# alipay/PainlessInferenceAcceleration

Hardware: NVIDIA H100
Metric: accepted tokens/sec @ Llama-2-7B 64-draft/8-branch; mean accepted len/step (higher is better)
Workload: dtype bf16

## Files before the change

painlessinferenceacceleration_b200/csrc/fused_ops.cu:

```cuda
#include <cuda_bf16.h>

#include "common.cuh"

namespace pia {
namespace fused {

__device__ __forceinline__ float bf(float x) { return __bfloat162float(__float2bfloat16_rn(x)); }

union Pack8 { uint4 u; __nv_bfloat16 h[8]; };

__device__ __forceinline__ Pack8 load_x8(const __nv_bfloat16 *x, const float *parts, int n_parts, long long part_stride,
                                         long long off) {
  Pack8 a;
  if (parts == nullptr) { a.u = *reinterpret_cast<const uint4 *>(x + off); return a; }
  float acc[8] = {0.f, 0.f, 0.f, 0.f, 0.f, 0.f, 0.f, 0.f};
  for (int s = 0; s < n_parts; ++s) {
    const float4 lo = *reinterpret_cast<const float4 *>(parts + s * part_stride + off);
    const float4 hi = *reinterpret_cast<const float4 *>(parts + s * part_stride + off + 4);
    acc[0] += lo.x; acc[1] += lo.y; acc[2] += lo.z; acc[3] += lo.w;
    acc[4] += hi.x; acc[5] += hi.y; acc[6] += hi.z; acc[7] += hi.w;
  }
#pragma unroll
  for (int j = 0; j < 8; ++j) a.h[j] = __float2bfloat16_rn(acc[j]);
  return a;
}

__global__ void __launch_bounds__(512) k_rmsnorm(const __nv_bfloat16 *x, const float *parts, int n_parts,
                                                 long long part_stride, const __nv_bfloat16 *res_in,
                                                 const __nv_bfloat16 *w, float eps, int hidden,
                                                 __nv_bfloat16 *res_out, __nv_bfloat16 *y) {
  __shared__ float red[16];
  pdl_launch_dependents();
  pdl_wait();
  const int row = blockIdx.x, tid = threadIdx.x;
  const int nvec = hidden >> 3;
  const long long row_off = (long long)row * hidden;
  const uint4 *rv = res_in ? reinterpret_cast<const uint4 *>(res_in + (long long)row * hidden) : nullptr;
  uint4 *rov = res_out ? reinterpret_cast<uint4 *>(res_out + (long long)row * hidden) : nullptr;
  float ss = 0.f;
  Pack8 keep[2];
  int cnt = 0;
  for (int v = tid; v < nvec; v += 512) {
    Pack8 a = load_x8(x, parts, n_parts, part_stride, row_off + v * 8);
    if (rv) {
      Pack8 r; r.u = rv[v];
#pragma unroll
      for (int j = 0; j < 8; ++j) a.h[j] = __float2bfloat16_rn(__bfloat162float(a.h[j]) + __bfloat162float(r.h[j]));
    }
    if (rov) rov[v] = a.u;
#pragma unroll
    for (int j = 0; j < 8; ++j) { const float f = __bfloat162float(a.h[j]); ss += f * f; }
    if (cnt < 2) keep[cnt] = a;
    ++cnt;
  }
#pragma unroll
  for (int o = 16; o > 0; o >>= 1) ss += __shfl_xor_sync(FULL, ss, o);
  if ((tid & 31) == 0) red[tid >> 5] = ss;
  __syncthreads();
  float tot = 0.f;
#pragma unroll
  for (int i = 0; i < 16; ++i) tot += red[i];
  const float inv = rsqrtf(tot / (float)hidden + eps);
  const uint4 *wv = reinterpret_cast<const uint4 *>(w);
  uint4 *yv = reinterpret_cast<uint4 *>(y + (long long)row * hidden);
  cnt = 0;
  for (int v = tid; v < nvec; v += 512) {
    Pack8 a;
    if (cnt < 2) a = keep[cnt];
    else {
      a = load_x8(x, parts, n_parts, part_stride, row_off + v * 8);
      if (rv) { Pack8 r; r.u = rv[v];
#pragma unroll
        for (int j = 0; j < 8; ++j) a.h[j] = __float2bfloat16_rn(__bfloat162float(a.h[j]) + __bfloat162float(r.h[j])); }
    }
    ++cnt;
    Pack8 ww; ww.u = wv[v];
    Pack8 o;
#pragma unroll
    for (int j = 0; j < 8; ++j) o.h[j] = __float2bfloat16_rn(__bfloat162float(ww.h[j]) * (__bfloat162float(a.h[j]) * inv));
    yv[v] = o.u;
  }
}

enum { ROPE_HALF = 0, ROPE_INTERLEAVED = 1, ROPE_HALF_F32 = 2 };
template <int kLayout>
__global__ void __launch_bounds__(256) k_rope_kv_append(const __nv_bfloat16 *qkv, const unsigned long long *mask,
                                                        int mask_words, pia_slots_t sl,
                                                        int hq, int hkv, int hd, const void *cos_t,
                                                        const void *sin_t, int max_pos, __nv_bfloat16 *q_out,
                                                        __nv_bfloat16 *kc, __nv_bfloat16 *vc, int max_seq,
                                                        int rotary_dim) {
  pdl_launch_dependents();
  pdl_wait();
  const int i = blockIdx.x;
  const int slot = i / sl.rows_per_slot, node = i % sl.rows_per_slot;
  const int n = sl.d_n[slot], P = sl.d_prefix_len[slot];
  const int pad_len = sl.d_pad_len ? sl.d_pad_len[slot] : 0;
  if (node >= n) return;
  kc += (long long)slot * sl.kv_slot_stride;
  vc += (long long)slot * sl.kv_slot_stride;
  int depth = -1;
  for (int w = 0; w < mask_words; ++w) depth += __popcll(mask[(long long)i * mask_words + w]);
  int pos = (P > pad_len ? P - pad_len : 0) + depth;
  if (pos < 0) pos = 0;
  if (pos >= max_pos) pos = max_pos - 1;
  const int half = hd >> 1, cpr = hd >> 3;
  const int row_elems = (hq + 2 * hkv) * hd;
  const __nv_bfloat16 *src = qkv + (long long)i * row_elems;
  const int cache_row = P + node;
  const int total = (hq + 2 * hkv) * cpr;
  for (int c = threadIdx.x; c < total; c += blockDim.x) {
    const int head = c / cpr, ch = c % cpr;
    const int d0 = ch * 8;
    Pack8 a; a.u = *reinterpret_cast<const uint4 *>(src + head * hd + d0);
    if (head < hq + hkv) {
      Pack8 o;
      const __nv_bfloat16 *cos_b = static_cast<const __nv_bfloat16 *>(cos_t);
      const __nv_bfloat16 *sin_b = static_cast<const __nv_bfloat16 *>(sin_t);
      if constexpr (kLayout == ROPE_INTERLEAVED) {
        o = a;
        if (d0 < rotary_dim) {
          const int rhalf = rotary_dim >> 1;
          union { uint2 u; __nv_bfloat16 h[4]; } cs, sn;
          cs.u = *reinterpret_cast<const uint2 *>(cos_b + (long long)pos * rhalf + (d0 >> 1));
          sn.u = *reinterpret_cast<const uint2 *>(sin_b + (long long)pos * rhalf + (d0 >> 1));
#pragma unroll
          for (int j = 0; j < 4; ++j) {
            const float x0 = __bfloat162float(a.h[2 * j]), x1 = __bfloat162float(a.h[2 * j + 1]);
            const float c = __bfloat162float(cs.h[j]), s = __bfloat162float(sn.h[j]);
            o.h[2 * j] = __float2bfloat16_rn(bf(x0 * c) + bf(-x1 * s));
            o.h[2 * j + 1] = __float2bfloat16_rn(bf(x1 * c) + bf(x0 * s));
          }
        }
      } else if constexpr (kLayout == ROPE_HALF_F32) {
        const int dp = d0 < half ? d0 + half : d0 - half;
        Pack8 b; b.u = *reinterpret_cast<const uint4 *>(src + head * hd + dp);
        const float *cf = static_cast<const float *>(cos_t) + (long long)pos * half + d0 % half;
        const float *sf = static_cast<const float *>(sin_t) + (long long)pos * half + d0 % half;
        float c[8], s[8];
        *reinterpret_cast<float4 *>(c) = *reinterpret_cast<const float4 *>(cf);
        *reinterpret_cast<float4 *>(c + 4) = *reinterpret_cast<const float4 *>(cf + 4);
        *reinterpret_cast<float4 *>(s) = *reinterpret_cast<const float4 *>(sf);
        *reinterpret_cast<float4 *>(s + 4) = *reinterpret_cast<const float4 *>(sf + 4);
#pragma unroll
        for (int j = 0; j < 8; ++j) {
          const float x = __bfloat162float(a.h[j]);
          const float r = d0 < half ? -__bfloat162float(b.h[j]) : __bfloat162float(b.h[j]);
          o.h[j] = __float2bfloat16_rn(__fadd_rn(__fmul_rn(x, c[j]), __fmul_rn(r, s[j])));
        }
      } else {
        const int dp = d0 < half ? d0 + half : d0 - half;
        Pack8 b; b.u = *reinterpret_cast<const uint4 *>(src + head * hd + dp);
        Pack8 cs, sn;
        const int f0 = d0 % half;
        cs.u = *reinterpret_cast<const uint4 *>(cos_b + (long long)pos * half + f0);
        sn.u = *reinterpret_cast<const uint4 *>(sin_b + (long long)pos * half + f0);
#pragma unroll
        for (int j = 0; j < 8; ++j) {
          const float x = __bfloat162float(a.h[j]);
          const float r = d0 < half ? -__bfloat162float(b.h[j]) : __bfloat162float(b.h[j]);
          o.h[j] = __float2bfloat16_rn(bf(x * __bfloat162float(cs.h[j])) + bf(r * __bfloat162float(sn.h[j])));
        }
      }
      if (head < hq) *reinterpret_cast<uint4 *>(q_out + ((long long)i * hq + head) * hd + d0) = o.u;
      else *reinterpret_cast<uint4 *>(kc + ((long long)(head - hq) * max_seq + cache_row) * hd + d0) = o.u;
    } else {
      *reinterpret_cast<uint4 *>(vc + ((long long)(head - hq - hkv) * max_seq + cache_row) * hd + d0) = a.u;
    }
  }
}

__global__ void __launch_bounds__(256) k_silu_mul(const __nv_bfloat16 *gu, int inter, __nv_bfloat16 *out) {
  pdl_launch_dependents();
  pdl_wait();
  const int row = blockIdx.y;
  const int v = blockIdx.x * 256 + threadIdx.x;
  if (v * 8 >= inter) return;
  Pack8 g, u, o;
  g.u = *reinterpret_cast<const uint4 *>(gu + (long long)row * 2 * inter + v * 8);
  u.u = *reinterpret_cast<const uint4 *>(gu + (long long)row * 2 * inter + inter + v * 8);
#pragma unroll
  for (int j = 0; j < 8; ++j) {
    const float x = __bfloat162float(g.h[j]);
    const float s = bf(x / (1.f + expf(-x)));
    o.h[j] = __float2bfloat16_rn(s * __bfloat162float(u.h[j]));
  }
  *reinterpret_cast<uint4 *>(out + (long long)row * inter + v * 8) = o.u;
}

__global__ void __launch_bounds__(256) k_embed_gather(const __nv_bfloat16 *table, const int *ids, const int *d_n,
                                                      int hidden, __nv_bfloat16 *out) {
  pdl_launch_dependents();
  pdl_wait();
  const int row = blockIdx.x;
  const int n = *d_n;
  const int nvec = hidden >> 3;
  uint4 *dst = reinterpret_cast<uint4 *>(out + (long long)row * hidden);
  if (row >= n) { for (int v = threadIdx.x; v < nvec; v += 256) dst[v] = make_uint4(0, 0, 0, 0); return; }
  const uint4 *src = reinterpret_cast<const uint4 *>(table + (long long)ids[row] * hidden);
  for (int v = threadIdx.x; v < nvec; v += 256) dst[v] = src[v];
}

}
}

using namespace pia;
using namespace pia::fused;

extern "C" int pia_rmsnorm(const void *d_x, const void *d_residual_in, const void *d_weight, float eps, int rows,
                           int hidden, void *d_residual_out, void *d_y, void *stream) {
  PIA_REQUIRE(d_x && d_weight && d_y && rows > 0 && hidden > 0 && hidden % 8 == 0, "bad rmsnorm arguments");
  PIA_CUDA_CHECK(launch_kernel(k_rmsnorm, dim3(rows), dim3(512), 0, (cudaStream_t)stream, (const __nv_bfloat16 *)d_x,
                              (const float *)nullptr, 0, 0ll, (const __nv_bfloat16 *)d_residual_in,
                              (const __nv_bfloat16 *)d_weight, eps, hidden, (__nv_bfloat16 *)d_residual_out,
                              (__nv_bfloat16 *)d_y));
  count_launch();
  return PIA_OK;
}

extern "C" int pia_rmsnorm_partials(const float *d_x_parts, int n_parts, int64_t part_stride, const void *d_residual_in,
                                    const void *d_weight, float eps, int rows, int hidden, void *d_residual_out,
                                    void *d_y, void *stream) {
  PIA_REQUIRE(d_x_parts && n_parts >= 1 && d_weight && d_y && rows > 0 && hidden > 0 && hidden % 8 == 0, "bad rmsnorm arguments");
  PIA_CUDA_CHECK(launch_kernel(k_rmsnorm, dim3(rows), dim3(512), 0, (cudaStream_t)stream,
                              (const __nv_bfloat16 *)nullptr, d_x_parts, n_parts, (long long)part_stride,
                              (const __nv_bfloat16 *)d_residual_in, (const __nv_bfloat16 *)d_weight, eps, hidden,
                              (__nv_bfloat16 *)d_residual_out, (__nv_bfloat16 *)d_y));
  count_launch();
  return PIA_OK;
}

template <int kLayout>
static int rope_kv_append(const void *d_qkv, const uint64_t *d_mask, int mask_words, const pia_slots_t *slots,
                          int n_q_heads, int n_kv_heads, int head_dim, const void *d_cos, const void *d_sin, int max_pos,
                          void *d_q_out, void *d_k_cache_layer, void *d_v_cache_layer, int max_seq, int rotary_dim,
                          void *stream) {
  PIA_REQUIRE(d_qkv && d_mask && slots && slots->d_n && slots->d_prefix_len && d_cos && d_sin && d_q_out &&
                  d_k_cache_layer && d_v_cache_layer, "null argument");
  PIA_REQUIRE(slots->batch >= 1 && slots->rows_per_slot >= 1 && slots->kv_slot_stride >= 0, "bad slot table");
  PIA_REQUIRE(head_dim % 16 == 0 && mask_words >= 1 && mask_words <= 2, "bad rope arguments");
  PIA_CUDA_CHECK(launch_kernel(k_rope_kv_append<kLayout>, dim3(slots->batch * slots->rows_per_slot), dim3(256), 0,
                              (cudaStream_t)stream, (const __nv_bfloat16 *)d_qkv, (const unsigned long long *)d_mask,
                              mask_words, *slots, n_q_heads, n_kv_heads, head_dim, d_cos, d_sin, max_pos,
                              (__nv_bfloat16 *)d_q_out,
                              (__nv_bfloat16 *)d_k_cache_layer, (__nv_bfloat16 *)d_v_cache_layer, max_seq, rotary_dim));
  count_launch();
  return PIA_OK;
}

extern "C" int pia_rope_kv_append(const void *d_qkv, const uint64_t *d_mask, int mask_words, const pia_slots_t *slots,
                                  int n_q_heads, int n_kv_heads, int head_dim, const void *d_cos, const void *d_sin,
                                  int max_pos, void *d_q_out, void *d_k_cache_layer, void *d_v_cache_layer, int max_seq,
                                  void *stream) {
  return rope_kv_append<ROPE_HALF>(d_qkv, d_mask, mask_words, slots, n_q_heads, n_kv_heads, head_dim, d_cos, d_sin,
                                   max_pos, d_q_out, d_k_cache_layer, d_v_cache_layer, max_seq, head_dim, stream);
}

extern "C" int pia_rope_f32_kv_append(const void *d_qkv, const uint64_t *d_mask, int mask_words, const pia_slots_t *slots,
                                      int n_q_heads, int n_kv_heads, int head_dim, const void *d_cos, const void *d_sin,
                                      int max_pos, void *d_q_out, void *d_k_cache_layer, void *d_v_cache_layer,
                                      int max_seq, void *stream) {
  return rope_kv_append<ROPE_HALF_F32>(d_qkv, d_mask, mask_words, slots, n_q_heads, n_kv_heads, head_dim, d_cos, d_sin,
                                       max_pos, d_q_out, d_k_cache_layer, d_v_cache_layer, max_seq, head_dim, stream);
}

extern "C" int pia_rope_interleaved_kv_append(const void *d_qkv, const uint64_t *d_mask, int mask_words,
                                              const pia_slots_t *slots, int n_q_heads, int n_kv_heads, int head_dim,
                                              const void *d_cos, const void *d_sin, int max_pos, void *d_q_out,
                                              void *d_k_cache_layer, void *d_v_cache_layer, int max_seq,
                                              int rotary_dim, void *stream) {
  PIA_REQUIRE(rotary_dim >= 8 && rotary_dim % 8 == 0 && rotary_dim <= head_dim,
              "bad rotary_dim: a positive multiple of 8, at most head_dim");
  return rope_kv_append<ROPE_INTERLEAVED>(d_qkv, d_mask, mask_words, slots, n_q_heads, n_kv_heads, head_dim, d_cos, d_sin, max_pos,
                              d_q_out, d_k_cache_layer, d_v_cache_layer, max_seq, rotary_dim, stream);
}

extern "C" int pia_silu_mul(const void *d_gate_up, int rows, int inter, void *d_out, void *stream) {
  PIA_REQUIRE(d_gate_up && d_out && rows > 0 && inter > 0 && inter % 8 == 0, "bad silu_mul arguments");
  dim3 grid((inter / 8 + 255) / 256, rows);
  PIA_CUDA_CHECK(launch_kernel(k_silu_mul, grid, dim3(256), 0, (cudaStream_t)stream, (const __nv_bfloat16 *)d_gate_up,
                              inter, (__nv_bfloat16 *)d_out));
  count_launch();
  return PIA_OK;
}

__global__ void __launch_bounds__(256) k_moe_combine(const __nv_bfloat16 *ye, const __nv_bfloat16 *w, int n_exp, int rows_cap,
                                                     int hidden, __nv_bfloat16 *out) {
  pdl_launch_dependents();
  pdl_wait();
  const int t = blockIdx.x;
  for (int v = threadIdx.x; v * 8 < hidden; v += blockDim.x) {
    Pack8 acc;
#pragma unroll
    for (int j = 0; j < 8; ++j) acc.h[j] = __float2bfloat16_rn(0.f);
    for (int e = 0; e < n_exp; ++e) {
      const float we = __bfloat162float(w[(long long)t * n_exp + e]);
      Pack8 y;
      y.u = *reinterpret_cast<const uint4 *>(ye + ((long long)e * rows_cap + t) * hidden + v * 8);
#pragma unroll
      for (int j = 0; j < 8; ++j)
        acc.h[j] = __float2bfloat16_rn(__bfloat162float(acc.h[j]) + bf(__bfloat162float(y.h[j]) * we));
    }
    *reinterpret_cast<uint4 *>(out + (long long)t * hidden + v * 8) = acc.u;
  }
}

extern "C" int pia_moe_combine(const void *d_expert_out, const void *d_weights, int n_experts, int rows, int rows_cap,
                               int hidden, void *d_out, void *stream) {
  PIA_REQUIRE(d_expert_out && d_weights && d_out && n_experts > 0 && rows > 0 && rows <= rows_cap && hidden % 8 == 0,
              "bad combine arguments");
  PIA_CUDA_CHECK(launch_kernel(k_moe_combine, dim3(rows), dim3(256), 0, (cudaStream_t)stream,
                              (const __nv_bfloat16 *)d_expert_out, (const __nv_bfloat16 *)d_weights, n_experts, rows_cap,
                              hidden, (__nv_bfloat16 *)d_out));
  count_launch();
  return PIA_OK;
}

__global__ void __launch_bounds__(256) k_moe_router(const __nv_bfloat16 *y, const __nv_bfloat16 *gate_w, int hidden,
                                                    int n_exp, int top_k, __nv_bfloat16 *dense) {
  __shared__ float s_logit[64];
  pdl_launch_dependents();
  pdl_wait();
  const int t = blockIdx.x, warp = threadIdx.x >> 5, lane = threadIdx.x & 31;
  const __nv_bfloat16 *yr = y + (long long)t * hidden;
  for (int e = warp; e < n_exp; e += 8) {
    const __nv_bfloat16 *wr = gate_w + (long long)e * hidden;
    float acc = 0.f;
    for (int v = lane; v * 8 < hidden; v += 32) {
      Pack8 a, w;
      a.u = *reinterpret_cast<const uint4 *>(yr + v * 8);
      w.u = *reinterpret_cast<const uint4 *>(wr + v * 8);
#pragma unroll
      for (int j = 0; j < 8; ++j) acc += __bfloat162float(a.h[j]) * __bfloat162float(w.h[j]);
    }
#pragma unroll
    for (int o = 16; o > 0; o >>= 1) acc += __shfl_xor_sync(FULL, acc, o);
    if (lane == 0) s_logit[e] = bf(acc);
  }
  __syncthreads();
  if (threadIdx.x == 0) {
    float mx = -INFINITY;
    for (int e = 0; e < n_exp; ++e) mx = fmaxf(mx, s_logit[e]);
    float den = 0.f, p[64];
    for (int e = 0; e < n_exp; ++e) { p[e] = expf(s_logit[e] - mx); den += p[e]; }
    for (int e = 0; e < n_exp; ++e) p[e] /= den;
    unsigned long long chosen = 0ull;
    float sum = 0.f;
    for (int k = 0; k < top_k; ++k) {
      int best = -1;
      for (int e = 0; e < n_exp; ++e)
        if (!((chosen >> e) & 1ull) && (best < 0 || p[e] > p[best])) best = e;
      chosen |= 1ull << best;
      sum += p[best];
    }
    for (int e = 0; e < n_exp; ++e)
      dense[(long long)t * n_exp + e] = __float2bfloat16_rn(((chosen >> e) & 1ull) ? p[e] / sum : 0.f);
  }
}

extern "C" int pia_moe_router(const void *d_y, const void *d_gate_weight, int rows, int hidden, int n_experts, int top_k,
                              void *d_dense_out, void *stream) {
  PIA_REQUIRE(d_y && d_gate_weight && d_dense_out && rows > 0 && hidden % 8 == 0 && n_experts >= 1 && n_experts <= 64 &&
                  top_k >= 1 && top_k <= n_experts, "bad router arguments");
  PIA_CUDA_CHECK(launch_kernel(k_moe_router, dim3(rows), dim3(256), 0, (cudaStream_t)stream, (const __nv_bfloat16 *)d_y,
                              (const __nv_bfloat16 *)d_gate_weight, hidden, n_experts, top_k, (__nv_bfloat16 *)d_dense_out));
  count_launch();
  return PIA_OK;
}

__global__ void __launch_bounds__(32) k_l2_prefetch(const char *base, long long n_ranges, long long stride,
                                                     long long range_bytes, int chunk, float bytes_per_ns) {
  const long long cpr = (range_bytes + chunk - 1) / chunk;
  const long long total = cpr * n_ranges;
  unsigned long long t0;
  asm volatile("mov.u64 %0, %%globaltimer;" : "=l"(t0));
  for (long long c = (long long)threadIdx.x * gridDim.x + blockIdx.x; c < total; c += (long long)blockDim.x * gridDim.x) {
    const long long k = c / n_ranges, r = c % n_ranges;
    const long long off = k * chunk;
    const long long left = range_bytes - off;
    const unsigned sz = (unsigned)(left < chunk ? left : chunk);
    if (bytes_per_ns > 0.f) {
      const unsigned long long due = t0 + (unsigned long long)((float)(c * chunk) / bytes_per_ns);
      unsigned long long now;
      asm volatile("mov.u64 %0, %%globaltimer;" : "=l"(now));
      while (now < due) {
        __nanosleep(64);
        asm volatile("mov.u64 %0, %%globaltimer;" : "=l"(now));
      }
    }
    asm volatile("cp.async.bulk.prefetch.L2.global [%0], %1;" ::"l"(base + r * stride + off), "r"(sz) : "memory");
  }
}

extern "C" int pia_l2_prefetch(const void *d_base, int64_t n_ranges, int64_t stride_bytes, int64_t range_bytes,
// ... 27 lines not shown
```

painlessinferenceacceleration_b200/csrc/gemm_ws.cu:

```cuda
#include <cuda.h>
#include <cuda_bf16.h>
#include <cuda_fp16.h>

#include <new>

#include "common.cuh"

namespace pia {
namespace gemm {

constexpr int BMW = 128;
constexpr int BK = 64;
constexpr int TOK = 64;
constexpr int NTHREADS = 288;
constexpr int PRODUCER_WARP = 8;
constexpr int W_BYTES = BMW * BK * 2, X_BYTES = TOK * BK * 2, STAGE_BYTES = W_BYTES + X_BYTES;
constexpr int XCH_BYTES = TOK * 64 * 2;
constexpr int smem_total(int nstage) { return nstage * STAGE_BYTES + 256 + XCH_BYTES + 1024; }
constexpr int ACC_OFF = 32 * 1024, ACC_LD = TOK + 4;
static_assert(ACC_OFF + BMW * ACC_LD * 4 <= 4 * STAGE_BYTES, "accumulator staging must fit in the pipeline stages");

__device__ __forceinline__ uint32_t smem_u32(const void *p) { return (uint32_t)__cvta_generic_to_shared(p); }
__device__ __forceinline__ void mbar_init(uint32_t bar, int count) {
  asm volatile("mbarrier.init.shared::cta.b64 [%0], %1;" ::"r"(bar), "r"(count));
}
__device__ __forceinline__ void mbar_arrive(uint32_t bar) {
  asm volatile("mbarrier.arrive.shared::cta.b64 _, [%0];" ::"r"(bar) : "memory");
}
__device__ __forceinline__ void mbar_expect_tx(uint32_t bar, uint32_t bytes) {
  asm volatile("mbarrier.arrive.expect_tx.shared::cta.b64 _, [%0], %1;" ::"r"(bar), "r"(bytes) : "memory");
}
__device__ __forceinline__ void mbar_wait(uint32_t bar, uint32_t parity) {
  uint32_t done;
  do {
    asm volatile(
        "{\n\t.reg .pred p;\n\t"
        "mbarrier.try_wait.parity.shared::cta.b64 p, [%1], %2;\n\t"
        "selp.u32 %0, 1, 0, p;\n\t}"
        : "=r"(done)
        : "r"(bar), "r"(parity)
        : "memory");
  } while (!done);
}
__device__ __forceinline__ void cluster_sync_all() {
  asm volatile("barrier.cluster.arrive.release.aligned;\n\tbarrier.cluster.wait.acquire.aligned;" ::: "memory");
}
__device__ __forceinline__ uint32_t map_to_cta(uint32_t local_smem_addr, uint32_t cta_rank) {
  uint32_t r;
  asm volatile("mapa.shared::cluster.u32 %0, %1, %2;" : "=r"(r) : "r"(local_smem_addr), "r"(cta_rank));
  return r;
}
__device__ __forceinline__ void st_cluster_f4(uint32_t addr, float a, float b, float c, float d) {
  asm volatile("st.shared::cluster.v4.f32 [%0], {%1, %2, %3, %4};" ::"r"(addr), "f"(a), "f"(b), "f"(c), "f"(d) : "memory");
}
__device__ __forceinline__ void tma_load_2d(uint32_t dst, const CUtensorMap *map, uint32_t bar, int c0, int c1) {
  asm volatile(
      "cp.async.bulk.tensor.2d.shared::cluster.global.mbarrier::complete_tx::bytes [%0], [%1, {%3, %4}], [%2];"
      ::"r"(dst), "l"(map), "r"(bar), "r"(c0), "r"(c1)
      : "memory");
}
__device__ __forceinline__ void tma_load_3d(uint32_t dst, const CUtensorMap *map, uint32_t bar, int c0, int c1, int c2) {
  asm volatile(
      "cp.async.bulk.tensor.3d.shared::cluster.global.mbarrier::complete_tx::bytes [%0], [%1, {%3, %4, %5}], [%2];"
      ::"r"(dst), "l"(map), "r"(bar), "r"(c0), "r"(c1), "r"(c2)
      : "memory");
}
__device__ __forceinline__ uint64_t kmajor_desc(uint32_t saddr) {
  uint64_t d = 0;
  d |= (uint64_t)((saddr >> 4) & 0x3FFF);
  d |= (uint64_t)1 << 16;
  d |= (uint64_t)(1024 >> 4) << 32;
  d |= (uint64_t)1 << 62;
  return d;
}
__device__ __forceinline__ void wgmma_fence() { asm volatile("wgmma.fence.sync.aligned;" ::: "memory"); }
__device__ __forceinline__ void wgmma_commit() { asm volatile("wgmma.commit_group.sync.aligned;" ::: "memory"); }
__device__ __forceinline__ void wgmma_wait_all() { asm volatile("wgmma.wait_group.sync.aligned 0;" ::: "memory"); }
__device__ __forceinline__ void fence_acc(float (&d)[32]) {
#pragma unroll
  for (int i = 0; i < 32; ++i) asm volatile("" : "+f"(d[i])::"memory");
}
__device__ __forceinline__ void wgmma_m64n64k16(float (&d)[32], uint64_t desc_a, uint64_t desc_b) {
  asm volatile(
      "{\n\t"
      "wgmma.mma_async.sync.aligned.m64n64k16.f32.bf16.bf16 "
      "{%0, %1, %2, %3, %4, %5, %6, %7, %8, %9, %10, %11, %12, %13, %14, %15, "
      "%16, %17, %18, %19, %20, %21, %22, %23, %24, %25, %26, %27, %28, %29, %30, %31}, %32, %33, 1, 1, 1, 0, 0;\n\t}"
      : "+f"(d[0]), "+f"(d[1]), "+f"(d[2]), "+f"(d[3]), "+f"(d[4]), "+f"(d[5]), "+f"(d[6]), "+f"(d[7]), "+f"(d[8]),
        "+f"(d[9]), "+f"(d[10]), "+f"(d[11]), "+f"(d[12]), "+f"(d[13]), "+f"(d[14]), "+f"(d[15]), "+f"(d[16]),
        "+f"(d[17]), "+f"(d[18]), "+f"(d[19]), "+f"(d[20]), "+f"(d[21]), "+f"(d[22]), "+f"(d[23]), "+f"(d[24]),
        "+f"(d[25]), "+f"(d[26]), "+f"(d[27]), "+f"(d[28]), "+f"(d[29]), "+f"(d[30]), "+f"(d[31])
      : "l"(desc_a), "l"(desc_b)
      : "memory");
}
__device__ __forceinline__ void mma_stage(float (&acc)[32], uint32_t wa, uint32_t xa) {
  wgmma_fence();
#pragma unroll
  for (int j = 0; j < BK / 16; ++j) wgmma_m64n64k16(acc, kmajor_desc(wa + j * 32), kmajor_desc(xa + j * 32));
  wgmma_commit();
  wgmma_wait_all();
  fence_acc(acc);
}
__device__ __forceinline__ int frag_row(int warp, int lane, int h) { return 16 * (warp & 3) + (lane >> 2) + 8 * h; }
__device__ __forceinline__ int frag_tok(int lane, int i) { return 8 * i + 2 * (lane & 3); }

struct Params {
  int N, K, n_split, chunks_per_split, n_chunks, rows, tiled;
  int groups, w_group_rows, x_group_chunks;
  long long out_group_stride;
  int cluster;
  int silu;
  int no_pdl;
  __nv_bfloat16 *out_bf16;
  float *out_f32;
};

template <int NSTAGE>
__global__ void __launch_bounds__(NTHREADS, NSTAGE <= 4 ? 2 : 1)
k_gemm_ws(const __grid_constant__ CUtensorMap map_w, const __grid_constant__ CUtensorMap map_x, Params p) {
  constexpr int SMEM_BAR = NSTAGE * STAGE_BYTES;
  extern __shared__ uint8_t smem_raw[];
  const uint32_t base = (smem_u32(smem_raw) + 1023u) & ~1023u;
  uint8_t *sm = smem_raw + (base - smem_u32(smem_raw));
  const int tid = threadIdx.x, warp = tid >> 5, lane = tid & 31;
  const uint32_t bar_full = base + SMEM_BAR, bar_empty = bar_full + 8 * NSTAGE;
  const int tile = p.cluster ? blockIdx.y : blockIdx.x, split = p.cluster ? blockIdx.x : blockIdx.y;
  const int n0 = tile * BMW;
  const int grp = blockIdx.z;
  const int xk0 = grp * p.x_group_chunks;
  const int c0 = split * p.chunks_per_split;
  int c1 = c0 + p.chunks_per_split;
  if (c1 > p.n_chunks) c1 = p.n_chunks;
  const int nch = c1 - c0;

  if (tid == 0) {
    for (int s = 0; s < NSTAGE; ++s) { mbar_init(bar_full + 8 * s, 1); mbar_init(bar_empty + 8 * s, 8); }
    asm volatile("fence.mbarrier_init.release.cluster;" ::: "memory");
  }
  __syncwarp();
  if (!p.no_pdl) pdl_launch_dependents();
  __syncthreads();

  if (warp == PRODUCER_WARP) {
    if (lane == 0) {
      auto load_w = [&](int i, int s) {
        const uint32_t wd = base + s * STAGE_BYTES;
        if (p.tiled) tma_load_3d(wd, &map_w, bar_full + 8 * s, 0, 0, tile * p.n_chunks + c0 + i);
        else tma_load_2d(wd, &map_w, bar_full + 8 * s, (c0 + i) * BK, grp * p.w_group_rows + n0);
      };
      const int pre = nch < NSTAGE ? nch : NSTAGE;
      for (int i = 0; i < pre; ++i) {
        mbar_expect_tx(bar_full + 8 * i, STAGE_BYTES);
        load_w(i, i);
      }
      pdl_wait();
      for (int i = 0; i < pre; ++i) tma_load_2d(base + i * STAGE_BYTES + W_BYTES, &map_x, bar_full + 8 * i, (xk0 + c0 + i) * BK, 0);
      for (int i = pre; i < nch; ++i) {
        const int s = i % NSTAGE, ph = (i / NSTAGE) & 1;
        mbar_wait(bar_empty + 8 * s, ph ^ 1);
        mbar_expect_tx(bar_full + 8 * s, STAGE_BYTES);
        load_w(i, s);
        tma_load_2d(base + s * STAGE_BYTES + W_BYTES, &map_x, bar_full + 8 * s, (xk0 + c0 + i) * BK, 0);
      }
    }
    __syncwarp();
    if (p.cluster) { cluster_sync_all(); cluster_sync_all(); }
    return;
  }

  pdl_wait();
  const int wg = warp >> 2;
  float acc[32];
#pragma unroll
  for (int j = 0; j < 32; ++j) acc[j] = 0.f;
  for (int i = 0; i < nch; ++i) {
    const int s = i % NSTAGE, ph = (i / NSTAGE) & 1;
    mbar_wait(bar_full + 8 * s, ph);
    const uint32_t wa = base + s * STAGE_BYTES, xa = wa + W_BYTES;
    mma_stage(acc, wa + wg * 64 * 128, xa);
    __syncwarp();
    if (lane == 0) mbar_arrive(bar_empty + 8 * s);
  }
  float *accs = reinterpret_cast<float *>(sm + ACC_OFF);
  asm volatile("bar.sync 2, 256;" ::: "memory");
#pragma unroll
  for (int h = 0; h < 2; ++h) {
    const int r = wg * 64 + frag_row(warp, lane, h);
#pragma unroll
    for (int i = 0; i < 8; ++i)
      *reinterpret_cast<float2 *>(accs + r * ACC_LD + frag_tok(lane, i)) = make_float2(acc[4 * i + 2 * h], acc[4 * i + 2 * h + 1]);
  }
  asm volatile("bar.sync 2, 256;" ::: "memory");
  if (wg == 1) {
    if (p.cluster) { cluster_sync_all(); cluster_sync_all(); }
    return;
  }

  const int q = warp;
  const int n = n0 + q * 32 + lane;
  uint32_t v[64];
  {
    const float4 *src = reinterpret_cast<const float4 *>(accs + (q * 32 + lane) * ACC_LD);
#pragma unroll
    for (int t = 0; t < 16; ++t) {
      const float4 a = src[t];
      v[4 * t] = __float_as_uint(a.x); v[4 * t + 1] = __float_as_uint(a.y);
      v[4 * t + 2] = __float_as_uint(a.z); v[4 * t + 3] = __float_as_uint(a.w);
    }
  }
  if (p.cluster) {
    const int cs = p.cluster, RS = BMW / cs;
    cluster_sync_all();
    {
      const int row = q * 32 + lane;
      const int owner = row / RS, rl = row % RS;
      const uint32_t dst = map_to_cta(base + (uint32_t)((split * 16) * RS + rl) * 16, owner);
#pragma unroll
      for (int tq = 0; tq < 16; ++tq)
        st_cluster_f4(dst + (uint32_t)(tq * RS) * 16, __uint_as_float(v[4 * tq]), __uint_as_float(v[4 * tq + 1]),
                      __uint_as_float(v[4 * tq + 2]), __uint_as_float(v[4 * tq + 3]));
    }
    cluster_sync_all();
    {
      const int e = warp * 32 + lane;
      const int rl = e % RS, tg = e / RS;
      const int qpt = RS / 8;
      const int n_out = n0 + split * RS + rl;
      const float4 *buf = reinterpret_cast<const float4 *>(sm);
      __nv_bfloat16 *ob = p.out_bf16 + grp * p.out_group_stride;
      if (n_out < p.N) {
        for (int tq = tg * qpt; tq < (tg + 1) * qpt; ++tq) {
          float4 a = buf[(0 * 16 + tq) * RS + rl];
          for (int src = 1; src < cs; ++src) {
            const float4 b = buf[(src * 16 + tq) * RS + rl];
            a.x += b.x; a.y += b.y; a.z += b.z; a.w += b.w;
          }
          const int t0 = 4 * tq;
          if (t0 < p.rows) ob[(long long)t0 * p.N + n_out] = __float2bfloat16_rn(a.x);
          if (t0 + 1 < p.rows) ob[(long long)(t0 + 1) * p.N + n_out] = __float2bfloat16_rn(a.y);
          if (t0 + 2 < p.rows) ob[(long long)(t0 + 2) * p.N + n_out] = __float2bfloat16_rn(a.z);
          if (t0 + 3 < p.rows) ob[(long long)(t0 + 3) * p.N + n_out] = __float2bfloat16_rn(a.w);
        }
      }
    }
  } else
  if (p.silu) {
    __nv_bfloat16 *xu = reinterpret_cast<__nv_bfloat16 *>(sm + SMEM_BAR + 256);
    __nv_bfloat16 *xg = xu + 32 * 64;
    const int rr = (q & 1) * 32 + lane;
    if (q >= 2) {
#pragma unroll
      for (int t = 0; t < 32; ++t) xu[t * 64 + rr] = __float2bfloat16_rn(__uint_as_float(v[t]));
    } else {
#pragma unroll
      for (int t = 0; t < 32; ++t) xg[t * 64 + rr] = __float2bfloat16_rn(__uint_as_float(v[32 + t]));
    }
    asm volatile("bar.sync 1, 128;" ::: "memory");
    const int col = tile * 64 + rr;
    const int inter = p.N >> 1;
    if (col < inter) {
      const int tb = q < 2 ? 0 : 32;
#pragma unroll
      for (int t = 0; t < 32; ++t) {
        if (tb + t < p.rows) {
          const float g = q < 2 ? __bfloat162float(__float2bfloat16_rn(__uint_as_float(v[t]))) : __bfloat162float(xg[t * 64 + rr]);
          const float u = q < 2 ? __bfloat162float(xu[t * 64 + rr]) : __bfloat162float(__float2bfloat16_rn(__uint_as_float(v[32 + t])));
          const float sg = __bfloat162float(__float2bfloat16_rn(g / (1.f + expf(-g))));
          p.out_bf16[(long long)(tb + t) * inter + col] = __float2bfloat16_rn(sg * u);
        }
      }
    }
  } else
  if (n < p.N) {
    if (p.n_split == 1) {
#pragma unroll
      for (int t = 0; t < TOK; ++t)
        if (t < p.rows) p.out_bf16[grp * p.out_group_stride + (long long)t * p.N + n] = __float2bfloat16_rn(__uint_as_float(v[t]));
    } else {
      float *o = p.out_f32 + (long long)split * TOK * p.N;
#pragma unroll
      for (int t = 0; t < TOK; ++t)
        if (t < p.rows) o[(long long)t * p.N + n] = __uint_as_float(v[t]);
    }
  }
}


struct SkParams {
  int N, n_tiles, n_chunks, rows, max_contrib;
  long long units;
  __nv_bfloat16 *out;
  float *ws;
  int *flags;
};

__device__ __forceinline__ long long sk_begin(long long b, long long U, int G) { return b * U / G; }
__device__ __forceinline__ int sk_cta_of(long long x, long long U, int G) {
  int b = (int)(x * G / U);
  while (b + 1 < G && sk_begin(b + 1, U, G) <= x) ++b;
  while (b > 0 && sk_begin(b, U, G) > x) --b;
  return b;
}

constexpr int SK_STAGES = 8;
constexpr int SK_SMEM_BAR = SK_STAGES * STAGE_BYTES;
constexpr int SK_SMEM_TOTAL = SK_SMEM_BAR + 256 + 1024;

__global__ void __launch_bounds__(NTHREADS, 1)
k_gemm_sk(const __grid_constant__ CUtensorMap map_w, const __grid_constant__ CUtensorMap map_x, SkParams p) {
  extern __shared__ uint8_t smem_raw[];
  const uint32_t base = (smem_u32(smem_raw) + 1023u) & ~1023u;
  const int tid = threadIdx.x, warp = tid >> 5, lane = tid & 31;
  const uint32_t bar_full = base + SK_SMEM_BAR, bar_empty = bar_full + 8 * SK_STAGES;
  const int G = gridDim.x, b = blockIdx.x;
  const long long u0 = sk_begin(b, p.units, G), u1 = sk_begin(b + 1, p.units, G);

  if (tid == 0) {
    for (int s = 0; s < SK_STAGES; ++s) { mbar_init(bar_full + 8 * s, 1); mbar_init(bar_empty + 8 * s, 8); }
    asm volatile("fence.mbarrier_init.release.cluster;" ::: "memory");
  }
  __syncwarp();
  pdl_launch_dependents();
  __syncthreads();
  pdl_wait();

  if (warp == PRODUCER_WARP) {
    if (lane == 0) {
      int i = 0;
      for (long long u = u0; u < u1; ++u, ++i) {
        const int tile = (int)(u / p.n_chunks), ch = (int)(u % p.n_chunks);
        const int s = i % SK_STAGES, ph = (i / SK_STAGES) & 1;
        mbar_wait(bar_empty + 8 * s, ph ^ 1);
        mbar_expect_tx(bar_full + 8 * s, STAGE_BYTES);
        const uint32_t wd = base + s * STAGE_BYTES, xd = wd + W_BYTES;
        tma_load_3d(wd, &map_w, bar_full + 8 * s, 0, 0, tile * p.n_chunks + ch);
// ... 614 lines not shown
```

painlessinferenceacceleration_b200/models/llama/modeling_llama.py:

```python
import glob
import json
import math
import os

import torch
from torch import nn

from ...common import ops
from ...common.pretrained_model import LookaheadPreTrainedModel


class LlamaRMSNorm(nn.Module):
    def __init__(self, hidden_size, eps=1e-6, device=None, dtype=None):
        super().__init__()
        self.weight = nn.Parameter(torch.ones(hidden_size, device=device, dtype=dtype))
        self.variance_epsilon = eps


class LlamaAttention(nn.Module):
    def __init__(self, cfg, device, dtype, qkv_bias=False):
        super().__init__()
        hd = cfg.hidden_size // cfg.num_attention_heads
        kv = getattr(cfg, 'num_key_value_heads', None) or cfg.num_attention_heads
        kw = dict(bias=False, device=device, dtype=dtype)
# ... 272 lines not shown
    def quantize_fp8(self):
        if self._fp8:
            return self
        self.fuse()
        for li, layer in enumerate(self.model.layers):
            for name, shape in self._fp8_weight_shapes(layer):
                if shape[-1] % 128 or shape[-2] % 128:
                    raise ValueError(f'layer {li} {name} {tuple(shape)}: fp8 weights need both dimensions divisible by 128')
        self._rt = None
        self.__dict__.pop('_tiled_weights', None)
        for layer in self.model.layers:
            self._quantize_layer(layer)
        self._fp8 = True
        return self

    def _quantize_layer(self, layer):
        a = layer.self_attn
        nq, nk = a.q_proj.weight.shape[0], a.k_proj.weight.shape[0]
        qkv = Fp8Linear(a.qkv_weight)
        a.qkv_fp8 = qkv
        a.q_proj = Fp8Rows(qkv, 0, nq, a.q_proj.bias)
        a.k_proj = Fp8Rows(qkv, nq, nq + nk, a.k_proj.bias)
        a.v_proj = Fp8Rows(qkv, nq + nk, qkv.shape[0], a.v_proj.bias)
        a.qkv_weight = None
        a.o_proj = Fp8Linear(a.o_proj.weight.data)
        self._quantize_mlp(layer)

    def _quantize_mlp(self, layer):
        m = layer.mlp
        ni = m.gate_proj.weight.shape[0]
        gu = Fp8Linear(m.gate_up_weight, interleaved=True)
        m.gate_up_fp8 = gu
        m.gate_proj, m.up_proj = Fp8Rows(gu, 0, ni), Fp8Rows(gu, ni, 2 * ni)
        m.gate_up_weight = None
        m.down_proj = Fp8Linear(m.down_proj.weight.data)

    @staticmethod
    def _fp8_split(w, n_sm):
        tiles, chunks = w.shape[-2] // 128, w.shape[-1] // 128
        want = (n_sm * 7) // 8
        if tiles >= want:
            return 1
        best = 1
        for s in (2, 4, 8):
            if chunks >= s and -(-chunks // -(-chunks // s)) == s:
                best = s
                if tiles * s >= want:
                    break
        return -best if best > 1 else 1

    def _fp8_plans(self, b):
        plans = getattr(b, 'fp8_plans', None)
        if plans is not None:
            return plans
        if os.environ.get('PIA_GEMM', '1') == '0' or 'PIA_GEMM_SET' in os.environ:
            raise ValueError('this model holds fp8 weights, which only the fp8 GEMM runs: PIA_GEMM=0 / PIA_GEMM_SET '
                             'do not apply')
        hid = self.config.hidden_size
        b.fp8_out = torch.zeros((b.rows, hid), dtype=torch.bfloat16, device=b.y.device)
        n_sm = torch.cuda.get_device_properties(b.y.device).multi_processor_count
        plans = {'layers': [self._layer_fp8_plans(layer, b, n_sm) for layer in self.model.layers]}
        b.fp8_plans = plans
        return plans

    def _attn_fp8_plans(self, layer, b, n_sm):
        a = layer.self_attn
        qkv, o = a.qkv_fp8, a.o_proj
        bias = a.qkv_bias.float() if a.qkv_bias is not None else None
        return {'qkv': ops.Gemm.fp8(qkv.qweight, qkv.scale, b.y, bias=bias, split_k=self._fp8_split(qkv, n_sm),
                                    out=b.qkv),
                'o': ops.Gemm.fp8(o.qweight, o.scale, b.attn, split_k=self._fp8_split(o, n_sm), out=b.fp8_out)}

    def _layer_fp8_plans(self, layer, b, n_sm):
        m = layer.mlp
        plans = self._attn_fp8_plans(layer, b, n_sm)
        if getattr(b, 'act', None) is None or b.act.shape[0] != b.rows:
            b.act = torch.zeros((b.rows, self.config.intermediate_size), dtype=torch.bfloat16, device=b.y.device)
        plans['gate_up_silu'] = ops.Gemm.fp8(m.gate_up_fp8.qweight, m.gate_up_fp8.scale, b.y, out=b.act).set_silu()
        plans['down'] = ops.Gemm.fp8(m.down_proj.qweight, m.down_proj.scale, b.act,
                                     split_k=self._fp8_split(m.down_proj, n_sm), out=b.fp8_out)
        return plans

    def geometry(self):
        c = self.config
        hd = c.hidden_size // c.num_attention_heads
        if getattr(c, 'head_dim', None) not in (None, hd):
            raise ValueError(f'config head_dim {c.head_dim} differs from hidden_size // num_attention_heads = {hd}; '
                             'only configs where the two are equal are supported')
        return dict(n_layers=c.num_hidden_layers, hidden=c.hidden_size, n_q_heads=c.num_attention_heads,
                    n_kv_heads=getattr(c, 'num_key_value_heads', None) or c.num_attention_heads, head_dim=hd,
                    inter=c.intermediate_size, vocab=c.vocab_size)

    def rope_tables(self, max_pos):
        c = self.config
        hd = c.hidden_size // c.num_attention_heads
        rp = getattr(c, 'rope_parameters', None) or {}
        theta = float(getattr(c, 'rope_theta', None) or rp.get('rope_theta', 10000.0))
        scaling = getattr(c, 'rope_scaling', None) or ({k: v for k, v in rp.items() if k != 'rope_theta'} if rp else None)
        rtype = (scaling or {}).get('rope_type', (scaling or {}).get('type', 'default')) if scaling else 'default'
        dev = self.device
        inv_freq = 1.0 / (theta ** (torch.arange(0, hd, 2, dtype=torch.int64).float().to(dev) / hd))
        pos = torch.arange(max_pos, device=dev).float()
        if rtype in (None, 'default'):
            pass
        elif rtype == 'linear':
            pos = pos / float(scaling['factor'])
        elif rtype == 'dynamic':
            factor, mpe = float(scaling['factor']), int(c.max_position_embeddings)
            if max_pos > mpe:
                base = theta * ((factor * max_pos / mpe) - (factor - 1)) ** (hd / (hd - 2))
                inv_freq = 1.0 / (base ** (torch.arange(0, hd, 2, dtype=torch.int64).float().to(dev) / hd))
        elif rtype == 'llama3':
            factor, low, high = float(scaling['factor']), float(scaling['low_freq_factor']), float(scaling['high_freq_factor'])
            old_ctx = scaling.get('original_max_position_embeddings') or c.max_position_embeddings
            low_freq_wavelen, high_freq_wavelen = old_ctx / low, old_ctx / high
            wavelen = 2 * math.pi / inv_freq
            inv_freq_llama = torch.where(wavelen > low_freq_wavelen, inv_freq / factor, inv_freq)
            smooth_factor = (old_ctx / wavelen - low) / (high - low)
            smoothed_inv_freq = (1 - smooth_factor) * inv_freq_llama / factor + smooth_factor * inv_freq_llama
            is_medium_freq = ~(wavelen < high_freq_wavelen) * ~(wavelen > low_freq_wavelen)
            inv_freq = torch.where(is_medium_freq, smoothed_inv_freq, inv_freq_llama)
        else:
            raise ValueError(f'Unknown RoPE scaling type {rtype}')
        freqs = pos[:, None] * inv_freq[None, :]
        return freqs.cos().to(torch.bfloat16).contiguous(), freqs.sin().to(torch.bfloat16).contiguous()

    def _gemm_plans(self, rt):
        plans = getattr(rt, 'gemm_plans', None)
        if plans is not None:
            return plans
        if self._fp8:
            self._fp8_plans(rt.decode_bufs)
            self._fp8_plans(rt.prefill_bufs)
            rt.gemm_plans = False
            return False
        import os
        if os.environ.get('PIA_GEMM', '1') == '0' or rt.max_nodes != 64:
            rt.gemm_plans = False
            return False
        b = rt.decode_bufs
        g = rt.g
        dev = b.y.device
        b.gu = torch.zeros((b.rows, 2 * g['inter']), dtype=torch.bfloat16, device=dev)
        b.act = torch.zeros((b.rows, g['inter']), dtype=torch.bfloat16, device=dev)
        plans = {'layers': []}
        for layer in self.model.layers:
            plans['layers'].append(self._layer_gemm_plans(layer, b))
        plans['lm_head'] = self._mk_gemm(self.lm_head.weight.data, b.y)
        rt.gemm_plans = plans
        return plans

    def _layer_gemm_plans(self, layer, b):
        import os
        want = os.environ.get('PIA_GEMM_SET', 'gate_up').split(',')
        if ('qkv' in want or 'qkv2' in want) and layer.self_attn.qkv_bias is not None:
            raise ValueError('PIA_GEMM_SET names qkv, but this model has QKV biases and k_gemm_ws has no bias epilogue')
        plans = {}
        if 'gate_up_silu' in want and layer.mlp.gate_up_weight.shape[0] % 256 == 0:
            cache = self.__dict__.setdefault('_tiled_weights', {})
            key = ('gate_up_silu', layer.mlp.gate_up_weight.data_ptr())
            if key not in cache:
                cache[key] = ops.tile_weight(ops.interleave_gate_up(layer.mlp.gate_up_weight))
            plans['gate_up_silu'] = ops.Gemm(cache[key], b.y, tiled=True).set_silu()
        elif 'gate_up' in want or 'gate_up_silu' in want:
            plans['gate_up'] = self._mk_gemm(layer.mlp.gate_up_weight, b.y)
        if 'qkv' in want:
            plans['qkv'] = self._mk_gemm(layer.self_attn.qkv_weight, b.y)
        sk = int(os.environ.get('PIA_GEMM_SPLIT', '-4'))
        if 'qkv2' in want:
            plans['qkv'] = self._mk_gemm(layer.self_attn.qkv_weight, b.y, split_k=-2)
        if 'o' in want:
            plans['o'] = self._mk_gemm(layer.self_attn.o_proj.weight.data, b.attn, split_k=sk)
        if 'down' in want and layer.mlp.down_proj.weight.shape[1] % 64 == 0 and layer.mlp.down_proj.weight.shape[1] >= 64 * abs(sk):
            plans['down'] = self._mk_gemm(layer.mlp.down_proj.weight.data, b.act, split_k=sk)
        for name in os.environ.get('PIA_GEMM_NOPDL', '').split(','):
            if name in plans:
                plans[name].set_pdl(False)
        return plans

    def _mk_gemm(self, w, x, split_k=1):
        if w.shape[0] % 128 == 0:
            cache = self.__dict__.setdefault('_tiled_weights', {})
            key = (w.data_ptr(), tuple(w.shape))
            if key not in cache:
                cache[key] = ops.tile_weight(w)
            return ops.Gemm(cache[key], x, split_k=split_k, tiled=True)
        return ops.Gemm(w.contiguous(), x, split_k=split_k)

    def _prefetch_cfg(self, rt):
        cfg = getattr(rt, 'prefetch_cfg', None)
        if cfg is None:
            import os
            spec = os.environ.get('PIA_PREFETCH', '0')
            v = [float(t) for t in spec.split(',')] if spec not in ('', '0') else []
            cfg = False
            if v and torch.cuda.is_available():
                v = (v + [0.0] * 4)[:4]
                cfg = dict(o=v[0], gate_up=v[1], down=v[2], rate=v[3], side=torch.cuda.Stream(device=self.device))
            rt.prefetch_cfg = cfg
        return cfg

    @staticmethod
    def _prefetch(pf, jobs):
        main = torch.cuda.current_stream()
        pf['side'].wait_stream(main)
        with torch.cuda.stream(pf['side']):
            for (t, frac, tile_bytes) in jobs:
                if frac <= 0:
                    continue
                total = t.numel() * t.element_size()
                if tile_bytes:
                    rb = max(16384, int(tile_bytes * min(frac, 1.0)) // 16384 * 16384)
                    ops.l2_prefetch(t, n_ranges=total // tile_bytes, stride_bytes=tile_bytes, range_bytes=min(rb, tile_bytes),
                                    gbytes_per_s=pf['rate'])
                else:
                    ops.l2_prefetch(t, range_bytes=int(total * min(frac, 1.0)) // 16 * 16, gbytes_per_s=pf['rate'])
        pf['dirty'] = True

    def _check_fused_attn(self):
        if self.rotary_interleaved and os.environ.get('PIA_ATTN_FUSED', '0') != '0':
            raise ValueError(f'{type(self).__name__} rotates interleaved pairs (GLM RoPE), which the fused attention '
                             'kernel does not: unset PIA_ATTN_FUSED')

    def _mlp(self, rt, layer, y, plans=None, pf=None, b=None):
        m = layer.mlp
        if plans:
            b = b if b is not None else rt.decode_bufs
            rows = y.shape[0]
            if 'gate_up_silu' in plans:
                plans['gate_up_silu'].run(rows, out=b.act)
            else:
                if 'gate_up' in plans:
                    plans['gate_up'].run(64, out=b.gu)
                else:
                    torch.mm(y, m.gate_up_weight.t(), out=b.gu)
                if pf:
                    self._prefetch(pf, [(m.down_proj.weight, pf['down'], 0)])
                ops.silu_mul(b.gu, b.act)
            if 'down' in plans:
                o = plans['down'].run(rows)
                return (o, None) if plans['down'].splits == 1 else (None, o)
            return torch.mm(b.act, m.down_proj.weight.t()), None
        gu = torch.mm(y, m.gate_up_weight.t())
        act = torch.empty((gu.shape[0], gu.shape[1] // 2), dtype=gu.dtype, device=gu.device)
        ops.silu_mul(gu, act)
        return torch.mm(act, m.down_proj.weight.t()), None

    def _verify_layers(self, rt, bufs=None, last_only=False):
        self.fuse()
        b = bufs if bufs is not None else rt.decode_bufs
        g = rt.g
        eps = self.config.rms_norm_eps
        ops.embed_gather(self.model.embed_tokens.weight, b.ids, b.n_total, b.h)
        if self._fp8:
            plans, rows = self._fp8_plans(b), b.rows
        else:
            plans, rows = (self._gemm_plans(rt) if b is rt.decode_bufs else False), 64
        pf = self._prefetch_cfg(rt) if plans and not self._fp8 else False
        fused_attn = b is rt.decode_bufs and os.environ.get('PIA_ATTN_FUSED', '0') != '0' and \
            (b.slots.batch == 1 or b.slots.kv_slot_stride != 0)
        if fused_attn:
            self._check_fused_attn()
        rotary_dim = g['rotary_dim'] if self.rotary_interleaved else None
        alibi = getattr(rt, 'alibi_slopes', None)
        x, parts, resid_in = b.h, None, None

        def norm(w):
            if parts is not None:
                ops.rmsnorm_partials(parts, resid_in, w, eps, b.resid, b.y)
            else:
                ops.rmsnorm(x, resid_in, w, eps, b.resid, b.y)

        def post_norm(w):
            if parts is not None:
                ops.rmsnorm_partials(parts, None, w, eps, None, b.post_norm)
            else:
                ops.rmsnorm(x, None, w, eps, None, b.post_norm)
            return b.post_norm, None

        for li, layer in enumerate(self.model.layers):
            lp = plans['layers'][li] if plans else None
            norm(layer.input_layernorm.weight)
            a = layer.self_attn
            if lp and 'qkv' in lp:
                lp['qkv'].run(rows, out=b.qkv)
            elif a.qkv_bias is not None:
                torch.addmm(a.qkv_bias, b.y, a.qkv_weight.t(), out=b.qkv)
            else:
                torch.mm(b.y, a.qkv_weight.t(), out=b.qkv)
            if pf and lp and 'gate_up' in lp:
                gw = lp['gate_up'].weight
                self._prefetch(pf, [(a.o_proj.weight, pf['o'], 0),
                                    (gw, pf['gate_up'], gw.shape[1] * gw.shape[2] * gw.shape[3] * 2 if gw.dim() == 4 else 0)])
            if fused_attn:
                rt.plan.forward_fused(li, b.qkv, b.mask, b.slots, rt.rope_cos, rt.rope_sin, b.attn)
            else:
                ops.rope_kv_append(b.qkv, b.mask, b.slots, g['n_q_heads'], g['n_kv_heads'], g['head_dim'], rt.rope_cos,
                                   rt.rope_sin, b.q, rt.k_layer(li, b.kv_slot), rt.v_layer(li, b.kv_slot), rt.max_seq,
                                   rotary_dim=rotary_dim)
                rt.plan.forward(li, b.q, b.mask, b.slots, b.attn, alibi_slopes=alibi)
            if lp and 'o' in lp:
                o = lp['o'].run(rows)
                x, parts, resid_in = (o, None, b.resid) if lp['o'].splits == 1 else (None, o, b.resid)
            else:
                x, parts, resid_in = torch.mm(b.attn, a.o_proj.weight.t()), None, b.resid
            if self.sandwich_norms:
                x, parts = post_norm(layer.post_self_attn_layernorm.weight)
# ... 19 lines not shown
```

Baseline: 561.7.

## Split rope blocks, add L2 evict-first hints, overlap wgmma stages, default fused SiLU

The rope/KV-append kernel gets a second grid dimension so each row's heads are spread across several blocks rather than one. The warp-specialized GEMM loads weights with an L2 evict_first cache hint and keeps one wgmma group in flight, releasing the previous stage's buffer only after the next stage is issued. The default GEMM set changes to the gate_up_silu plan with interleaved tiled weights and a fused SiLU epilogue. These are several unrelated changes. The deferred buffer release delays stage reuse, and the fused SiLU path needs a different weight layout.

```diff
diff --git a/painlessinferenceacceleration_b200/csrc/fused_ops.cu b/painlessinferenceacceleration_b200/csrc/fused_ops.cu
--- a/painlessinferenceacceleration_b200/csrc/fused_ops.cu
+++ b/painlessinferenceacceleration_b200/csrc/fused_ops.cu
@@ -109,7 +109,7 @@
   const __nv_bfloat16 *src = qkv + (long long)i * row_elems;
   const int cache_row = P + node;
   const int total = (hq + 2 * hkv) * cpr;
-  for (int c = threadIdx.x; c < total; c += blockDim.x) {
+  for (int c = blockIdx.y * blockDim.x + threadIdx.x; c < total; c += blockDim.x * gridDim.y) {
     const int head = c / cpr, ch = c % cpr;
     const int d0 = ch * 8;
     Pack8 a; a.u = *reinterpret_cast<const uint4 *>(src + head * hd + d0);
@@ -239,7 +239,8 @@
                   d_k_cache_layer && d_v_cache_layer, "null argument");
   PIA_REQUIRE(slots->batch >= 1 && slots->rows_per_slot >= 1 && slots->kv_slot_stride >= 0, "bad slot table");
   PIA_REQUIRE(head_dim % 16 == 0 && mask_words >= 1 && mask_words <= 2, "bad rope arguments");
-  PIA_CUDA_CHECK(launch_kernel(k_rope_kv_append<kLayout>, dim3(slots->batch * slots->rows_per_slot), dim3(256), 0,
+  const int chunk_blocks = ((n_q_heads + 2 * n_kv_heads) * (head_dim / 8) + 255) / 256;
+  PIA_CUDA_CHECK(launch_kernel(k_rope_kv_append<kLayout>, dim3(slots->batch * slots->rows_per_slot, chunk_blocks), dim3(256), 0,
                               (cudaStream_t)stream, (const __nv_bfloat16 *)d_qkv, (const unsigned long long *)d_mask,
                               mask_words, *slots, n_q_heads, n_kv_heads, head_dim, d_cos, d_sin, max_pos,
                               (__nv_bfloat16 *)d_q_out,
diff --git a/painlessinferenceacceleration_b200/csrc/gemm_ws.cu b/painlessinferenceacceleration_b200/csrc/gemm_ws.cu
--- a/painlessinferenceacceleration_b200/csrc/gemm_ws.cu
+++ b/painlessinferenceacceleration_b200/csrc/gemm_ws.cu
@@ -65,6 +65,24 @@
       ::"r"(dst), "l"(map), "r"(bar), "r"(c0), "r"(c1), "r"(c2)
       : "memory");
 }
+__device__ __forceinline__ uint64_t l2_evict_first_policy() {
+  uint64_t pol;
+  asm volatile("createpolicy.fractional.L2::evict_first.b64 %0, 1.0;" : "=l"(pol));
+  return pol;
+}
+__device__ __forceinline__ void tma_load_2d_hint(uint32_t dst, const CUtensorMap *map, uint32_t bar, int c0, int c1, uint64_t pol) {
+  asm volatile(
+      "cp.async.bulk.tensor.2d.shared::cluster.global.mbarrier::complete_tx::bytes.L2::cache_hint [%0], [%1, {%3, %4}], [%2], %5;"
+      ::"r"(dst), "l"(map), "r"(bar), "r"(c0), "r"(c1), "l"(pol)
+      : "memory");
+}
+__device__ __forceinline__ void tma_load_3d_hint(uint32_t dst, const CUtensorMap *map, uint32_t bar, int c0, int c1, int c2,
+                                                 uint64_t pol) {
+  asm volatile(
+      "cp.async.bulk.tensor.3d.shared::cluster.global.mbarrier::complete_tx::bytes.L2::cache_hint [%0], [%1, {%3, %4, %5}], [%2], %6;"
+      ::"r"(dst), "l"(map), "r"(bar), "r"(c0), "r"(c1), "r"(c2), "l"(pol)
+      : "memory");
+}
 __device__ __forceinline__ uint64_t kmajor_desc(uint32_t saddr) {
   uint64_t d = 0;
   d |= (uint64_t)((saddr >> 4) & 0x3FFF);
@@ -76,6 +94,7 @@
 __device__ __forceinline__ void wgmma_fence() { asm volatile("wgmma.fence.sync.aligned;" ::: "memory"); }
 __device__ __forceinline__ void wgmma_commit() { asm volatile("wgmma.commit_group.sync.aligned;" ::: "memory"); }
 __device__ __forceinline__ void wgmma_wait_all() { asm volatile("wgmma.wait_group.sync.aligned 0;" ::: "memory"); }
+__device__ __forceinline__ void wgmma_wait_1() { asm volatile("wgmma.wait_group.sync.aligned 1;" ::: "memory"); }
 __device__ __forceinline__ void fence_acc(float (&d)[32]) {
 #pragma unroll
   for (int i = 0; i < 32; ++i) asm volatile("" : "+f"(d[i])::"memory");
@@ -143,10 +162,11 @@
 
   if (warp == PRODUCER_WARP) {
     if (lane == 0) {
+      const uint64_t pol = l2_evict_first_policy();
       auto load_w = [&](int i, int s) {
         const uint32_t wd = base + s * STAGE_BYTES;
-        if (p.tiled) tma_load_3d(wd, &map_w, bar_full + 8 * s, 0, 0, tile * p.n_chunks + c0 + i);
-        else tma_load_2d(wd, &map_w, bar_full + 8 * s, (c0 + i) * BK, grp * p.w_group_rows + n0);
+        if (p.tiled) tma_load_3d_hint(wd, &map_w, bar_full + 8 * s, 0, 0, tile * p.n_chunks + c0 + i, pol);
+        else tma_load_2d_hint(wd, &map_w, bar_full + 8 * s, (c0 + i) * BK, grp * p.w_group_rows + n0, pol);
       };
       const int pre = nch < NSTAGE ? nch : NSTAGE;
       for (int i = 0; i < pre; ++i) {
@@ -176,11 +196,17 @@
   for (int i = 0; i < nch; ++i) {
     const int s = i % NSTAGE, ph = (i / NSTAGE) & 1;
     mbar_wait(bar_full + 8 * s, ph);
-    const uint32_t wa = base + s * STAGE_BYTES, xa = wa + W_BYTES;
-    mma_stage(acc, wa + wg * 64 * 128, xa);
+    const uint32_t wa = base + s * STAGE_BYTES + wg * 64 * 128, xa = base + s * STAGE_BYTES + W_BYTES;
+    wgmma_fence();
+#pragma unroll
+    for (int j = 0; j < BK / 16; ++j) wgmma_m64n64k16(acc, kmajor_desc(wa + j * 32), kmajor_desc(xa + j * 32));
+    wgmma_commit();
+    wgmma_wait_1();
     __syncwarp();
-    if (lane == 0) mbar_arrive(bar_empty + 8 * s);
-  }
+    if (i > 0 && lane == 0) mbar_arrive(bar_empty + 8 * ((i - 1) % NSTAGE));
+  }
+  wgmma_wait_all();
+  fence_acc(acc);
   float *accs = reinterpret_cast<float *>(sm + ACC_OFF);
   asm volatile("bar.sync 2, 256;" ::: "memory");
 #pragma unroll
diff --git a/painlessinferenceacceleration_b200/models/llama/modeling_llama.py b/painlessinferenceacceleration_b200/models/llama/modeling_llama.py
--- a/painlessinferenceacceleration_b200/models/llama/modeling_llama.py
+++ b/painlessinferenceacceleration_b200/models/llama/modeling_llama.py
@@ -448,7 +448,7 @@
 
     def _layer_gemm_plans(self, layer, b):
         import os
-        want = os.environ.get('PIA_GEMM_SET', 'gate_up').split(',')
+        want = os.environ.get('PIA_GEMM_SET', 'gate_up_silu').split(',')
         if ('qkv' in want or 'qkv2' in want) and layer.self_attn.qkv_bias is not None:
             raise ValueError('PIA_GEMM_SET names qkv, but this model has QKV biases and k_gemm_ws has no bias epilogue')
         plans = {}
```

New measurement: 578.0 (median of 6 runs). 1.03x the previous value.
